# c0gent/hbbft

Hardware: AMD Instinct MI355X
Metric: verified BLS sig shares/sec (whole node) + combine latency, N=64 f=21 (higher is better)
Workload: dtype u32 limbs (Fp, 14x28-bit); 1 GPU; ThresholdSign share verification, BASELINE configs[1]; batch_per_gpu=65536, streams=2, documents_per_gpu=1024, n_nodes=64, f=21, pairing_impl=auto, parallelism=shard-by-batch x1

## Files before the change

### hbbft_amd/csrc/pfp.hpp

```cpp
#pragma once
#include "sfp.hpp"
#include "words.hpp"

#ifndef HP_INV_MODE
#define HP_INV_MODE 0
#endif

#define HP_D __device__ __forceinline__

namespace hbs {

constexpr int DPP_SWAP = 0xB1;
constexpr int DPP_EVEN = 0xA0;
constexpr int DPP_ODD = 0xF5;

HP_D bool lp_even() { return (threadIdx.x & 1) == 0; }
template <int CTRL>
HP_D int32_t dpp(int32_t v) {
  return __builtin_amdgcn_mov_dpp(v, CTRL, 0xF, 0xF, true);
}
template <int CTRL>
HP_D Fp dpp_fp(const Fp& a) {
  Fp r;
#pragma unroll
  for (int i = 0; i < NL; i++) r.l[i] = dpp<CTRL>(a.l[i]);
  return r;
}

HS_MULFN Fp h_mul_l(HS_P14(x), HS_P14(y)) {
  const Fp a = {{HS_L14(x)}};
  const Fp b = {{HS_L14(y)}};
  const int32_t sm = lp_even() ? -1 : 0;
  int32_t Y[NL], W[NL], Z[NL];
#pragma unroll
  for (int i = 0; i < NL; i++) {
    Y[i] = dpp<DPP_EVEN>(b.l[i]);
    W[i] = dpp<DPP_ODD>(b.l[i]);
    Z[i] = (dpp<DPP_SWAP>(a.l[i]) ^ sm) - sm;
  }
  int32_t m[NL];
  int64_t acc = 0;
  Fp r;
#pragma unroll
  for (int k = 0; k < NL; k++) {
#pragma unroll
    for (int i = 0; i <= k; i++) {
      acc += (int64_t)a.l[i] * Y[k - i];
      acc += (int64_t)Z[i] * W[k - i];
    }
#pragma unroll
    for (int i = 0; i < k; i++) acc += (int64_t)m[i] * (int32_t)P_L[k - i];
    m[k] = mont_digit(acc);
    acc += (int64_t)m[k] * (int32_t)P_L[0];
    acc >>= 28;
  }
#pragma unroll
  for (int k = NL; k < 2 * NL - 1; k++) {
#pragma unroll
    for (int i = k - NL + 1; i < NL; i++) {
      acc += (int64_t)a.l[i] * Y[k - i];
      acc += (int64_t)Z[i] * W[k - i];
      acc += (int64_t)m[i] * (int32_t)P_L[k - i];
    }
    r.l[k - NL] = (int32_t)acc & MASK28;
    acc >>= 28;
  }
  r.l[NL - 1] = (int32_t)acc;
  return r;
}

HP_D Fp h_mul(const Fp& a, const Fp& b) { return h_mul_l(HS_E14(a), HS_E14(b)); }

HP_D Fp h_sqr(const Fp& a) {
  const bool ev = lp_even();
  const Fp pa = dpp_fp<DPP_SWAP>(a);
  Fp x, y;
#pragma unroll
  for (int i = 0; i < NL; i++) {
    x.l[i] = pa.l[i] + (ev ? a.l[i] : pa.l[i]);
    y.l[i] = a.l[i] - (ev ? pa.l[i] : 0);
  }
  return fp_mul(x, y);
}

HP_D Fp h_mul_xi(const Fp& a) {
  const int32_t sm = lp_even() ? -1 : 0;
  const Fp pa = dpp_fp<DPP_SWAP>(a);
  Fp r;
#pragma unroll
  for (int i = 0; i < NL; i++) r.l[i] = a.l[i] + ((pa.l[i] ^ sm) - sm);
  fp_norm(r);
  return r;
}
HP_D Fp h_conj(const Fp& a) {
  const Fp n = fp_neg(a);
  return lp_even() ? a : n;
}
HP_D Fp h_zero() { return fp_zero(); }
HP_D Fp h_one() { return lp_even() ? fp_one() : fp_zero(); }
HP_D Fp h_const(const uint32_t (&c0)[NL], const uint32_t (&c1)[NL]) {
  Fp r;
  const bool ev = lp_even();
#pragma unroll
  for (int i = 0; i < NL; i++) r.l[i] = (int32_t)(ev ? c0[i] : c1[i]);
  return r;
}
HP_D bool lp_both(bool v) { return (v ? 1 : 0) & dpp<DPP_SWAP>(v ? 1 : 0); }
HP_D bool h_is_zero(const Fp& a) { return lp_both(fp_is_zero(a)); }
constexpr int INV_PAIR = 8;
template <int N>
HP_D void lp_inv_uniform(const uint32_t* y, const uint32_t* mod, uint32_t* out) {
  static_assert(N <= 15, "words_reduce_32m");
  const bool ev = lp_even();
  uint32_t mine[N], other[N], co[N + 1];
#pragma unroll
  for (int i = 0; i < N; i++) {
    mine[i] = ev ? y[i] : mod[i];
    other[i] = ev ? mod[i] : y[i];
    co[i] = 0;
  }
  co[N] = 0;
  co[0] = ev ? 1u : 0u;
  uint32_t inv = mod[0];
  for (int k = 0; k < 5; k++) inv *= 2u - mod[0] * inv;
  const uint32_t minv = 0u - inv;
  const int rounds = (2 * hb::words_bitlen<N>(mod) - 1 + 30) / 31;
#pragma unroll 1
  for (int r = 0; r < rounds; r++) {
    const uint64_t am = hb::words_approx<N>(mine, hb::words_len2<N>(mine, other));
    const uint64_t ao = (uint64_t)(uint32_t)dpp<DPP_SWAP>((int32_t)(uint32_t)am) |
                        ((uint64_t)(uint32_t)dpp<DPP_SWAP>((int32_t)(uint32_t)(am >> 32)) << 32);
    uint64_t ab = ev ? am : ao, bb = ev ? ao : am;
    uint32_t c0 = ev ? 1u : 0u, c1 = ev ? 0u : 1u;
#pragma unroll 1
    for (int j = 0; j < 31; j++) {
      uint32_t odd;
      bool sw;
      hb::words_divstep_ab(ab, bb, odd, sw);
      hb::words_divstep_col(c0, c1, odd, sw);
    }
    uint32_t km, ks, sm, ss;
    hb::words_fac_split(ev ? c0 : c1, km, ks);
    hb::words_fac_split(ev ? c1 : c0, sm, ss);
    {
      uint32_t t[N + 2], k[N + 2], row[N + 1];
      hb::words_mul_sm<N, false>(mine, sm, ss, t);
#pragma unroll
      for (int i = 0; i < N + 2; i++) t[i] = (uint32_t)dpp<DPP_SWAP>((int32_t)t[i]);
      hb::words_mul_sm<N, false>(mine, km, ks, k);
      uint64_t c = 0;
#pragma unroll
      for (int i = 0; i < N + 2; i++) {
        c += (uint64_t)k[i] + t[i];
        t[i] = (uint32_t)c;
        c >>= 32;
      }
#pragma unroll
      for (int i = 0; i <= N; i++) row[i] = (t[i] >> 31) | (t[i + 1] << 1);
      const uint32_t fl = hb::words_abs<N + 1>(row);
      ks ^= fl;
      ss ^= (uint32_t)dpp<DPP_SWAP>((int32_t)fl);
#pragma unroll
      for (int i = 0; i < N; i++) {
        mine[i] = row[i];
        other[i] = (uint32_t)dpp<DPP_SWAP>((int32_t)row[i]);
      }
    }
    {
      uint32_t t[N + 2], w[N + 2];
      hb::words_mul_sm<N, true>(co, sm, ss, t);
#pragma unroll
      for (int i = 0; i < N + 2; i++) t[i] = (uint32_t)dpp<DPP_SWAP>((int32_t)t[i]);
      const uint32_t xe = 0u - (co[N] >> 31);
      const uint32_t k0 = km & ks;
      const uint64_t q = (uint64_t)(((k0 + (co[0] ^ ks) * km + t[0]) * minv) & 0x7fffffffu);
      uint64_t c = k0;
#pragma unroll
      for (int i = 0; i < N + 2; i++) {
        const uint32_t xi = (i <= N ? co[i] : xe) ^ ks;
        c += (uint64_t)xi * km;
        if (i < N) c += q * mod[i];
        c += t[i];
        w[i] = (uint32_t)c;
        c >>= 32;
      }
#pragma unroll
      for (int i = 0; i <= N; i++) co[i] = (w[i] >> 31) | (w[i + 1] << 1);
    }
  }
  const uint32_t mine_one = hb::words_is_one<N>(mine) ? 1u : 0u;
  const uint32_t part_one = (uint32_t)dpp<DPP_SWAP>((int32_t)mine_one);
  const bool one = (ev ? part_one : mine_one) != 0;
  uint32_t v[N + 1];
#pragma unroll
  for (int i = 0; i <= N; i++) {
    const uint32_t pv = (uint32_t)dpp<DPP_SWAP>((int32_t)co[i]);
    v[i] = ev ? pv : co[i];
  }
  hb::words_reduce_32m<N>(v, mod);
#pragma unroll
  for (int i = 0; i < N; i++) out[i] = one ? v[i] : 0u;
}

template <int MODE = 0>
HP_D Fp h_inv_vartime(const Fp& a) {
  const Fp s = fp_sqr(a);
  const Fp n = fp_add(s, dpp_fp<DPP_SWAP>(s));
  uint32_t w[12], p[12], r[12];
  fp_to_words(n, w);
  uint32_t nz = 0;
#pragma unroll
  for (int i = 0; i < 12; i++) nz |= w[i];
  if (nz == 0) return fp_zero();
#pragma unroll
  for (int i = 0; i < 12; i++) p[i] = hb::PM2_W[i];
  p[0] += 2;
  if ((MODE & INV_PAIR) != 0)
    lp_inv_uniform<12>(w, p, r);
  else
    hb::words_inv_vartime<12, MODE>(w, p, r);
  return h_conj(fp_mul(a, fp_from_words(r)));
}

template <int M, int K>
HP_D Fp fp_red_mk(const Fp& t, const Fp& a) {
  const int64_t top = (int64_t)t.l[NL - 1] * M + (int64_t)K * a.l[NL - 1];
  const int32_t q = (int32_t)((top * QINV) >> 32);
  Fp r;
  int64_t acc = 0;
#pragma unroll
  for (int i = 0; i < NL - 1; i++) {
    acc += (int64_t)t.l[i] * M + (int64_t)K * a.l[i] - (int64_t)q * (int32_t)P_L[i];
    r.l[i] = (int32_t)acc & MASK28;
    acc >>= 28;
  }
  r.l[NL - 1] = (int32_t)(acc + top - (int64_t)q * (int32_t)P_L[NL - 1]);
  return r;
}
HP_D Fp fp_red_l(const Fp& t) { return fp_red_mk<1, 0>(t, t); }
HP_D Fp fp_red_124(const Fp& a, const Fp& b, const Fp& c) {
  const int32_t top = a.l[NL - 1] + 2 * b.l[NL - 1] + 4 * c.l[NL - 1];
  const int32_t q = (int32_t)(((int64_t)top * QINV) >> 32);
  Fp r;
  int64_t acc = 0;
#pragma unroll
  for (int i = 0; i < NL - 1; i++) {
    acc += (int64_t)(a.l[i] + 2 * b.l[i] + 4 * c.l[i]) - (int64_t)q * (int32_t)P_L[i];
    r.l[i] = (int32_t)acc & MASK28;
    acc >>= 28;
  }
  r.l[NL - 1] = (int32_t)(acc + top - (int64_t)q * (int32_t)P_L[NL - 1]);
  return r;
}
HP_D Fp fp_lin3(const Fp& a, int k1, const Fp& b, int k2, const Fp& c) {
  Fp r;
#pragma unroll
  for (int i = 0; i < NL; i++) r.l[i] = a.l[i] + k1 * b.l[i] + k2 * c.l[i];
  fp_norm(r);
  return r;
}
HP_D Fp h_add_xi_l(const Fp& s, const Fp& t) {
  const int32_t sm = lp_even() ? -1 : 0;
  const Fp pt = dpp_fp<DPP_SWAP>(t);
  Fp r;
#pragma unroll
  for (int i = 0; i < NL; i++) r.l[i] = s.l[i] + t.l[i] + ((pt.l[i] ^ sm) - sm);
  return r;
}
HP_D Fp fp_sub2l(const Fp& a, const Fp& b, const Fp& c) {
  Fp r;
#pragma unroll
  for (int i = 0; i < NL; i++) r.l[i] = a.l[i] - b.l[i] - c.l[i];
  return r;
}

HP_D Fp h_xi_l(const Fp& t) {
  const int32_t sm = lp_even() ? -1 : 0;
  const Fp pt = dpp_fp<DPP_SWAP>(t);
  Fp r;
#pragma unroll
  for (int i = 0; i < NL; i++) r.l[i] = t.l[i] + ((pt.l[i] ^ sm) - sm);
  return r;
}

struct H6 { Fp c0, c1, c2; };
struct H12 { H6 c0, c1; };

HP_D H6 h6_zero() { return {h_zero(), h_zero(), h_zero()}; }
HP_D H6 h6_one() { return {h_one(), h_zero(), h_zero()}; }
HP_D H6 h6_add(const H6& a, const H6& b) { return {fp_add(a.c0, b.c0), fp_add(a.c1, b.c1), fp_add(a.c2, b.c2)}; }
HP_D H6 h6_sub(const H6& a, const H6& b) { return {fp_sub(a.c0, b.c0), fp_sub(a.c1, b.c1), fp_sub(a.c2, b.c2)}; }
HP_D H6 h6_neg(const H6& a) { return {fp_neg(a.c0), fp_neg(a.c1), fp_neg(a.c2)}; }
HP_D H6 h6_red(const H6& a) { return {fp_reduce(a.c0), fp_reduce(a.c1), fp_reduce(a.c2)}; }
HP_D H6 h6_mul_v(const H6& a) { return {h_mul_xi(a.c2), a.c0, a.c1}; }

HP_D H6 h6_mul(const H6& a, const H6& b) {
  const Fp v1 = h_mul(a.c1, b.c1);
  const Fp v2 = h_mul(a.c2, b.c2);
  const Fp d0 = fp_sub2l(h_mul(fp_addl(a.c1, a.c2), fp_add(b.c1, b.c2)), v1, v2);
  const Fp v0 = h_mul(a.c0, b.c0);
  const Fp c0 = fp_red_l(h_add_xi_l(v0, d0));
  const Fp c1 = fp_red_l(h_add_xi_l(fp_sub2l(h_mul(fp_addl(a.c0, a.c1), fp_add(b.c0, b.c1)), v0, v1), v2));
  const Fp c2 = fp_red_l(fp_addl(fp_sub2l(h_mul(fp_addl(a.c0, a.c2), fp_add(b.c0, b.c2)), v0, v2), v1));
  return {c0, c1, c2};
}
HP_D H6 h6_mul6(const H6& a, const H6& b) {
  Fp c2, m, e, k, h;
  {
    const Fp sa = fp_add(a.c0, a.c2);
    const Fp p1 = h_mul(fp_addl(sa, a.c1), fp_lin3(b.c0, 1, b.c1, 1, b.c2));
    const Fp pm = h_mul(fp_subl(sa, a.c1), fp_lin3(b.c0, -1, b.c1, 1, b.c2));
    const Fp p0 = h_mul(a.c0, b.c0);
    const Fp pi = h_mul(a.c2, b.c2);
    const Fp xpi = h_xi_l(pi);
    Fp w;
#pragma unroll
    for (int i = 0; i < NL; i++) {
      w.l[i] = p1.l[i] + pm.l[i] - 2 * p0.l[i] - 2 * pi.l[i];
      m.l[i] = 3 * (p0.l[i] - p1.l[i]) - pm.l[i];
      e.l[i] = p1.l[i] - pm.l[i];
      k.l[i] = p0.l[i] - 2 * xpi.l[i];
      h.l[i] = 2 * pi.l[i] + xpi.l[i];
    }
    c2 = fp_red_mk<3, 0>(w, w);
  }
  const Fp t = fp_addl(h_mul(fp_red_124(a.c0, a.c1, a.c2), fp_lin3(b.c0, 2, b.c1, 4, b.c2)), m);
  const Fp c0 = fp_red_mk<1, 6>(h_xi_l(t), k);
  Fp g;
#pragma unroll
  for (int i = 0; i < NL; i++) g.l[i] = 3 * e.l[i] - t.l[i];
  const Fp c1 = fp_red_mk<1, 6>(g, h);
  return {c0, c1, c2};
}
HP_D H6 h6_inv(const H6& a) {
  const Fp c0 = fp_reduce(fp_sub(h_sqr(a.c0), h_mul_xi(h_mul(a.c1, a.c2))));
  const Fp c1 = fp_reduce(fp_sub(h_mul_xi(h_sqr(a.c2)), h_mul(a.c0, a.c1)));
  const Fp c2 = fp_reduce(fp_sub(h_sqr(a.c1), h_mul(a.c0, a.c2)));
  const Fp t = fp_reduce(fp_add(h_mul(a.c0, c0), h_mul_xi(fp_add(h_mul(a.c2, c1), h_mul(a.c1, c2)))));
  const Fp ti = fp_reduce(h_inv_vartime<HP_INV_MODE>(t));
  return {h_mul(c0, ti), h_mul(c1, ti), h_mul(c2, ti)};
}

HP_D H12 h12_one() { return {h6_one(), h6_zero()}; }
HP_D H12 h12_conj(const H12& a) { return {a.c0, h6_neg(a.c1)}; }
HP_D H12 h12_red(const H12& a) { return {h6_red(a.c0), h6_red(a.c1)}; }
HP_D H12 h12_kcomb(const H6& t0, const H6& t1, const H6& s) {
  return {{fp_red_l(h_add_xi_l(t0.c0, t1.c2)), fp_red_l(fp_addl(t0.c1, t1.c0)), fp_red_l(fp_addl(t0.c2, t1.c1))},
          {fp_red_l(fp_sub2l(s.c0, t0.c0, t1.c0)), fp_red_l(fp_sub2l(s.c1, t0.c1, t1.c1)),
           fp_red_l(fp_sub2l(s.c2, t0.c2, t1.c2))}};
}

template <int S = 1>
HP_D H6 h6_mul_12(const H6& x, const Fp& b1, const Fp& b2) {
  const Fp u = h_mul(x.c1, b1);
  const Fp w = h_mul(x.c2, b2);
  const Fp d0 = h_xi_l(fp_sub2l(h_mul(fp_addl(x.c1, x.c2), fp_add(b1, b2)), u, w));
  const Fp c0 = fp_red_mk<S, 0>(d0, d0);
  const Fp d1 = h_add_xi_l(h_mul(x.c0, b1), w);
  const Fp c1 = fp_red_mk<S, 0>(d1, d1);
  const Fp d2 = fp_addl(h_mul(x.c0, b2), u);
  const Fp c2 = fp_red_mk<S, 0>(d2, d2);
  return {c0, c1, c2};
}

HP_D const H6& h6_of(const H6& a) { return a; }
template <class F>
HP_D auto h6_of(const F& f) -> decltype(f()) { return f(); }

template <class G>
HP_D H12 h12_mul(const H12& a, const H12& b) {
  H6 t0, t1;
  G::mul6x2(a.c0, b.c0, a.c1, b.c1, t0, t1);
  const H6 s = G::mul6(h6_add(a.c0, a.c1), h6_add(b.c0, b.c1));
  return h12_kcomb(t0, t1, s);
}
template <class G>
HP_D H12 h12_sqr(const H12& a) {
  H6 t, s;
  const auto a1 = [&]() HS_LAMBDA { return h6_add(a.c0, a.c1); };
  const auto b1 = [&]() HS_LAMBDA { return h6_red(h6_add(a.c0, h6_mul_v(a.c1))); };
  G::miller_mul6x2(a.c0, a.c1, a1, b1, t, s);
  return {{fp_red_l(h_add_xi_l(fp_subl(s.c0, t.c0), fp_subl(fp_zero(), t.c2))), fp_red_l(fp_sub2l(s.c1, t.c1, t.c0)),
           fp_red_l(fp_sub2l(s.c2, t.c2, t.c1))},
          {fp_red_l(fp_addl(t.c0, t.c0)), fp_red_l(fp_addl(t.c1, t.c1)), fp_red_l(fp_addl(t.c2, t.c2))}};
}
template <class G>
HP_D H12 h12_mul_lines(const H12& f, const Fp& a0, const Fp& a1, const Fp& a4, const Fp& b0, const Fp& b1,
                       const Fp& b4, bool first = false) {
  H6 C0, t0, t1;
  Fp c11, c12;
  G::line_product(a0, a1, a4, b0, b1, b4, C0, c11, c12);
  if (first) return {C0, {h_zero(), c11, c12}};
  G::miller_mul6x2_12(f.c0, C0, f.c1, c11, c12, t0, t1);
  const H6 s = G::miller_mul6(h6_add(f.c0, f.c1), {C0.c0, fp_add(C0.c1, c11), fp_add(C0.c2, c12)});
  return h12_kcomb(t0, t1, s);
}
template <class G>
HP_D H12 h12_inv(const H12& a) {
  H6 s0, s1, r0, r1;
  G::mul6x2(a.c0, a.c0, a.c1, a.c1, s0, s1);
  const H6 t = h6_red(h6_sub(h6_red(s0), h6_red(h6_mul_v(h6_red(s1)))));
  const H6 ti = h6_red(h6_inv(t));
  G::mul6x2(a.c0, ti, a.c1, ti, r0, r1);
  return h12_red({r0, h6_neg(r1)});
}

#define HP_FROB1(K) h_const(hb::FROB1_##K##_C0, hb::FROB1_##K##_C1)
HP_D H12 h12_frob1(const H12& f) {
  H12 r;
  r.c0.c0 = h_conj(f.c0.c0);
  r.c1.c0 = h_mul(h_conj(f.c1.c0), HP_FROB1(1));
  r.c0.c1 = h_mul(h_conj(f.c0.c1), HP_FROB1(2));
  r.c1.c1 = h_mul(h_conj(f.c1.c1), HP_FROB1(3));
  r.c0.c2 = h_mul(h_conj(f.c0.c2), HP_FROB1(4));
  r.c1.c2 = h_mul(h_conj(f.c1.c2), HP_FROB1(5));
  return h12_red(r);
}
HP_D H12 h12_frob2(const H12& f) {
  H12 r;
  r.c0.c0 = f.c0.c0;
  r.c1.c0 = fp_mul(f.c1.c0, fp_const(hb::FROB2_1_C0));
  r.c0.c1 = fp_mul(f.c0.c1, fp_const(hb::FROB2_2_C0));
  r.c1.c1 = fp_mul(f.c1.c1, fp_const(hb::FROB2_3_C0));
  r.c0.c2 = fp_mul(f.c0.c2, fp_const(hb::FROB2_4_C0));
  r.c1.c2 = fp_mul(f.c1.c2, fp_const(hb::FROB2_5_C0));
  return r;
}

HP_D H12 h12_cyclo_sqr(const H12& f) {
  const Fp& a0 = f.c0.c0; const Fp& a2 = f.c0.c1; const Fp& a4 = f.c0.c2;
  const Fp& a1 = f.c1.c0; const Fp& a3 = f.c1.c1; const Fp& a5 = f.c1.c2;
  H12 r;
  {
    const Fp s0 = h_sqr(a0), s3 = h_sqr(a3), s03 = h_sqr(fp_add(a0, a3));
    r.c0.c0 = fp_red_mk<3, -2>(h_add_xi_l(s0, s3), a0);
    r.c1.c1 = fp_red_mk<3, 2>(fp_sub2l(s03, s0, s3), a3);
  }
  {
    const Fp s1 = h_sqr(a1), s4 = h_sqr(a4), s14 = h_sqr(fp_add(a1, a4));
    r.c0.c1 = fp_red_mk<3, -2>(h_add_xi_l(s1, s4), a2);
    r.c1.c2 = fp_red_mk<3, 2>(fp_sub2l(s14, s1, s4), a5);
  }
  {
    const Fp s2 = h_sqr(a2), s5 = h_sqr(a5), s25 = h_sqr(fp_add(a2, a5));
    r.c0.c2 = fp_red_mk<3, -2>(h_add_xi_l(s2, s5), a4);
    r.c1.c0 = fp_red_mk<3, 2>(h_add_xi_l(fp_zero(), fp_sub2l(s25, s2, s5)), a1);
  }
  return r;
}

struct HC { Fp a1, a2, a4, a5; };

HP_D HC hc_compress(const H12& f) { return {f.c1.c0, f.c0.c1, f.c0.c2, f.c1.c2}; }
HP_D HC hc_sqr(const HC& c) {
  HC r;
  {
    const Fp s1 = h_sqr(c.a1), s4 = h_sqr(c.a4), s14 = h_sqr(fp_add(c.a1, c.a4));
    r.a2 = fp_red_mk<3, -2>(h_add_xi_l(s1, s4), c.a2);
    r.a5 = fp_red_mk<3, 2>(fp_sub2l(s14, s1, s4), c.a5);
  }
  {
    const Fp s2 = h_sqr(c.a2), s5 = h_sqr(c.a5), s25 = h_sqr(fp_add(c.a2, c.a5));
    r.a4 = fp_red_mk<3, -2>(h_add_xi_l(s2, s5), c.a4);
    r.a1 = fp_red_mk<3, 2>(h_add_xi_l(fp_zero(), fp_sub2l(s25, s2, s5)), c.a1);
  }
  return r;
}
HP_D Fp hc_denom(const Fp& a1) { return fp_lin(4, a1, 0, a1); }
HP_D H12 hc_decompress(const HC& c, const Fp& di) {
  const Fp s5 = h_sqr(c.a5), s2 = h_sqr(c.a2);
  Fp t = h_xi_l(s5);
#pragma unroll
  for (int i = 0; i < NL; i++) t.l[i] += 3 * s2.l[i];
  const Fp a3 = h_mul(fp_red_mk<1, -2>(t, c.a4), di);
  const Fp u = fp_addl(fp_lin(2, h_sqr(a3), -3, h_mul(c.a4, c.a2)), h_mul(c.a1, c.a5));
  const Fp a0 = fp_red_l(h_add_xi_l(h_one(), u));
  return {{a0, c.a2, c.a4}, {c.a1, a3, c.a5}};
}

HP_D bool h12_is_one(const H12& f) {
  bool ok = fp_is_zero(fp_sub(f.c0.c0, h_one()));
  ok = ok && fp_is_zero(f.c0.c1) && fp_is_zero(f.c0.c2);
  ok = ok && fp_is_zero(f.c1.c0) && fp_is_zero(f.c1.c1) && fp_is_zero(f.c1.c2);
  return lp_both(ok);
}

struct HJac { Fp x, y, z; };
struct HLine { Fp c0, c1, c4; };

struct HProj { Fp x, y, z; };

HP_D HLine h_dbl_step_h(HProj& T) {
  const Fp C = h_sqr(T.z);
  const Fp YZ = h_sqr(fp_add(T.y, T.z));
  const Fp B = h_sqr(T.y);
  const Fp H = fp_sub(fp_sub(YZ, B), C);
  const Fp E = fp_red_mk<12, 0>(h_xi_l(C), C);
  const Fp A = h_mul(T.x, T.y);
  const Fp S = h_sqr(T.x);
  HLine l;
  l.c0 = fp_red_mk<1, -1>(B, E);
  l.c1 = fp_lin(-3, S, 0, S);
  l.c4 = H;
  const Fp Bm = fp_lin(1, B, -3, E);
  const Fp Bp = fp_lin(1, B, 3, E);
  T.x = h_mul(fp_addl(A, A), Bm);
  const Fp EE = h_sqr(E);
  T.y = fp_red_mk<1, -12>(h_sqr(Bp), EE);
  const Fp BH = h_mul(fp_addl(B, B), H);
  T.z = fp_red_mk<2, 0>(BH, BH);
  return l;
}

HP_D HLine h_add_step_h(HProj& T, const Fp& xQ, const Fp& yQ) {
  const Fp th = fp_sub(T.y, h_mul(yQ, T.z));
  const Fp la = fp_sub(T.x, h_mul(xQ, T.z));
  HLine l;
  l.c0 = fp_reduce(fp_sub(h_mul(th, xQ), h_mul(la, yQ)));
  l.c1 = fp_neg(th);
  l.c4 = la;
  const Fp C = h_sqr(th);
  const Fp D = h_sqr(la);
  const Fp E = h_mul(la, D);
  const Fp F = h_mul(T.z, C);
  const Fp G = h_mul(T.x, D);
  const Fp H = fp_lin(1, fp_addl(E, F), -2, G);
  const Fp X3 = h_mul(la, H);
  T.y = fp_reduce(fp_sub(h_mul(th, fp_sub(G, H)), h_mul(E, T.y)));
  T.z = h_mul(T.z, E);
  T.x = X3;
  return l;
}

template <class PT>
struct SideStateT {
  Fp xP, yP;
  bool act;
  bool qinf;
  uint32_t q;
  PT T;
};

template <bool GEN, class ST>
HP_D Fp side_xP(const ST& st) { return GEN ? fp_const(hb::G1X_M) : st.xP; }
template <bool GEN, class ST>
HP_D Fp side_yP(const ST& st, bool negate) {
  return GEN ? (negate ? fp_neg(fp_const(hb::G1Y_M)) : fp_const(hb::G1Y_M)) : st.yP;
}

struct NoPark {
  HP_D explicit NoPark(uint32_t*) {}
  template <class ST>
  HP_D void init(const ST&, const ST&) const {}
  template <int SIDE, class ST, class F>
  HP_D HLine walk(ST& st, const F& f) const { return f(st.T); }
  template <int SIDE, class ST>
  HP_D Fp xP(const ST& st) const { return st.xP; }
  template <int SIDE, class ST>
  HP_D Fp yP(const ST& st) const { return st.yP; }
};

constexpr int PARK_WORDS = 72;
constexpr int park_fit(int used, bool need, int words) { return need && used + words <= PARK_WORDS ? used : -1; }
typedef volatile __attribute__((address_space(3))) uint32_t* ParkCol;

HP_D void park_put(ParkCol c, int slot, const Fp& a) {
#pragma unroll
  for (int i = 0; i < NL; i++) c[(slot + i) * 256] = (uint32_t)a.l[i];
}
HP_D Fp park_get(ParkCol c, int slot) {
  Fp r;
#pragma unroll
  for (int i = 0; i < NL; i++) r.l[i] = (int32_t)c[(slot + i) * 256];
  return r;
}

template <bool W1, bool W2, int GEN>
struct PairPark {
  static constexpr int TW = 3 * NL, PW = 2 * NL;
  static constexpr int T_B = park_fit(0, W2, TW);
  static constexpr int U1 = T_B < 0 ? 0 : TW;
  static constexpr int T_A = park_fit(U1, W1, TW);
  static constexpr int U2 = U1 + (T_A < 0 ? 0 : TW);
  static constexpr int P_A = park_fit(U2, GEN != 1, PW);
  static constexpr int U3 = U2 + (P_A < 0 ? 0 : PW);
  static constexpr int P_B = park_fit(U3, GEN != 2, PW);
  template <int SIDE>
  static constexpr int t_slot() { return SIDE == 0 ? T_A : T_B; }
  template <int SIDE>
  static constexpr int p_slot() { return SIDE == 0 ? P_A : P_B; }

  ParkCol col;
  HP_D explicit PairPark(uint32_t* c) : col((ParkCol)c) {}

  template <int SIDE>
  HP_D void put_T(const HProj& T) const {
    park_put(col, t_slot<SIDE>(), T.x);
    park_put(col, t_slot<SIDE>() + NL, T.y);
    park_put(col, t_slot<SIDE>() + 2 * NL, T.z);
  }
  template <int SIDE, class ST>
  HP_D void init_side(const ST& st) const {
    if constexpr (t_slot<SIDE>() >= 0) put_T<SIDE>(st.T);
    if constexpr (p_slot<SIDE>() >= 0) {
      park_put(col, p_slot<SIDE>(), st.xP);
      park_put(col, p_slot<SIDE>() + NL, st.yP);
    }
  }
  template <class ST>
  HP_D void init(const ST& A, const ST& B) const {
    init_side<0>(A);
    init_side<1>(B);
  }
  template <int SIDE, class ST, class F>
  HP_D HLine walk(ST& st, const F& f) const {
    if constexpr (t_slot<SIDE>() < 0) {
      return f(st.T);
    } else {
      HProj T;
      T.z = park_get(col, t_slot<SIDE>() + 2 * NL);
      T.y = park_get(col, t_slot<SIDE>() + NL);
      T.x = park_get(col, t_slot<SIDE>());
      const HLine l = f(T);
      put_T<SIDE>(T);
      return l;
    }
  }
  template <int SIDE, class ST>
  HP_D Fp xP(const ST& st) const {
    if constexpr (p_slot<SIDE>() < 0) return st.xP; else return park_get(col, p_slot<SIDE>());
  }
  template <int SIDE, class ST>
  HP_D Fp yP(const ST& st) const {
    if constexpr (p_slot<SIDE>() < 0) return st.yP; else return park_get(col, p_slot<SIDE>() + NL);
  }
};

struct LanePair {
  static constexpr int LANES = 2;
  static HP_D bool leader() { return lp_even(); }
  static HP_D bool value_writer() { return true; }
  using Walk = HProj;
  static HP_D HLine dbl_step(HProj& T) { return h_dbl_step_h(T); }
  static HP_D HLine add_step(HProj& T, const Fp& xQ, const Fp& yQ) { return h_add_step_h(T, xQ, yQ); }

  static HP_D H6 mul6(const H6& a, const H6& b) { return h6_mul(a, b); }
  template <class A1, class B1>
  static HP_D void mul6x2(const H6& a0, const H6& b0, const A1& a1, const B1& b1, H6& r0, H6& r1) {
    r0 = h6_mul(a0, b0);
    r1 = h6_mul(h6_of(a1), h6_of(b1));
  }
  static HP_D void mul6x2_12(const H6& a0, const H6& b0, const H6& a1, const Fp& c1, const Fp& c2, H6& r0, H6& r1) {
    r0 = h6_mul(a0, b0);
    r1 = h6_mul_12(a1, c1, c2);
  }
  static constexpr int MILLER_SCALE = 6;
  static HP_D H6 miller_mul6(const H6& a, const H6& b) { return h6_mul6(a, b); }
  template <class A1, class B1>
  static HP_D void miller_mul6x2(const H6& a0, const H6& b0, const A1& a1, const B1& b1, H6& r0, H6& r1) {
    r0 = h6_mul6(a0, b0);
    r1 = h6_mul6(h6_of(a1), h6_of(b1));
  }
  static HP_D void miller_mul6x2_12(const H6& a0, const H6& b0, const H6& a1, const Fp& c1, const Fp& c2, H6& r0,
                                    H6& r1) {
    r0 = h6_mul6(a0, b0);
    r1 = h6_mul_12<MILLER_SCALE>(a1, c1, c2);
  }
  template <bool W1, bool W2>
  static constexpr bool first_line() { return W1 || W2; }
  static HP_D void line_product(const Fp& a0, const Fp& a1, const Fp& a4, const Fp& b0, const Fp& b1, const Fp& b4,
                                H6& C0, Fp& c11, Fp& c12) {
    const Fp a0b0 = h_mul(a0, b0);
    const Fp a1b1 = h_mul(a1, b1);
    const Fp a4b4 = h_mul(a4, b4);
    c11 = fp_red_l(fp_sub2l(h_mul(fp_addl(a0, a4), fp_add(b0, b4)), a0b0, a4b4));
    c12 = fp_red_l(fp_sub2l(h_mul(fp_addl(a1, a4), fp_add(b1, b4)), a1b1, a4b4));
    C0 = {fp_red_l(h_add_xi_l(a0b0, a4b4)), fp_red_l(fp_sub2l(h_mul(fp_addl(a0, a1), fp_add(b0, b1)), a0b0, a1b1)),
          a1b1};
  }
  static HP_D H12 cyclo_sqr(const H12& f) { return h12_cyclo_sqr(f); }
  static HP_D H12 frob1(const H12& f) { return h12_frob1(f); }
  static HP_D H12 frob2(const H12& f) { return h12_frob2(f); }

  template <bool W1, bool W2, int GEN>
  using Park = PairPark<W1, W2, GEN>;

  template <bool GEN, int SIDE, class ST, class PK>
  static HP_D HLine line_at_p(const HLine& l, const ST& st, bool negate, const PK& pk) {
    HLine e;
    e.c0 = st.act ? l.c0 : h_one();
    const Fp c1 = fp_mul(l.c1, GEN ? side_xP<true>(st) : pk.template xP<SIDE>(st));
    e.c1 = st.act ? c1 : fp_zero();
    const Fp c4 = fp_mul(l.c4, GEN ? side_yP<true>(st, negate) : pk.template yP<SIDE>(st));
    e.c4 = st.act ? c4 : fp_zero();
    return e;
  }
  template <bool G1, bool G2, bool WALK_FIRST, class RA, class RB, class ST, class PK>
  static HP_D void lines_at_p(const RA& raw_a, const RB& raw_b, const ST& A, const ST& B, bool neg2, HLine& la,
                              HLine& lb, const PK& pk) {
    if constexpr (WALK_FIRST) {
      lb = line_at_p<G2, 1>(raw_b(), B, neg2, pk);
      la = line_at_p<G1, 0>(raw_a(), A, false, pk);
    } else {
      la = line_at_p<G1, 0>(raw_a(), A, false, pk);
      lb = line_at_p<G2, 1>(raw_b(), B, neg2, pk);
    }
  }
};

HP_D void h_g2_load(const uint32_t* __restrict__ w, Fp& x, Fp& y) {
  const int o = lp_even() ? 0 : 12;
  x = fp_from_words(w + o);
  y = fp_from_words(w + 24 + o);
}
HP_D bool words_zero(const uint32_t* __restrict__ w, int n) {
  uint32_t o = 0;
  for (int k = 0; k < n; k++) o |= w[k];
  return o == 0;
}

}
```

Measured before the change: 3.863 million shares/s.

## Fuse Fp4 squaring triples into one interleaved Montgomery product in cyclotomic squaring

```diff
diff --git a/hbbft_amd/csrc/pfp.hpp b/hbbft_amd/csrc/pfp.hpp
--- a/hbbft_amd/csrc/pfp.hpp
+++ b/hbbft_amd/csrc/pfp.hpp
@@ -82,6 +82,90 @@
   }
   return fp_mul(x, y);
 }
+
+#ifndef HP_SQR4
+#define HP_SQR4 1
+#endif
+#if HP_SQR4
+typedef int32_t V28 __attribute__((ext_vector_type(2 * NL)));
+
+HS_MULFN V28 h_sqr4_l(HS_P14(x), HS_P14(y)) {
+  const Fp a = {{HS_L14(x)}};
+  const Fp b = {{HS_L14(y)}};
+  const int32_t sm = lp_even() ? -1 : 0;
+  int32_t xa[NL], ya[NL], xb[NL], yb[NL], xs[NL], ys[NL];
+#pragma unroll
+  for (int i = 0; i < NL; i++) {
+    const int32_t pa = dpp<DPP_SWAP>(a.l[i]), pb = dpp<DPP_SWAP>(b.l[i]);
+    xa[i] = dpp<DPP_EVEN>(a.l[i]) + pa;
+    ya[i] = a.l[i] - (pa & sm);
+    xb[i] = dpp<DPP_EVEN>(b.l[i]) + pb;
+    yb[i] = b.l[i] - (pb & sm);
+    xs[i] = xa[i] + xb[i];
+    ys[i] = ya[i] + yb[i];
+  }
+  int32_t mA[NL], mC[NL], A[NL], C[NL];
+  int64_t cb = 0, ra = 0, rc = 0;
+#pragma unroll
+  for (int k = 0; k < 2 * NL - 1; k++) {
+#pragma unroll
+    for (int i = (k < NL ? 0 : k - NL + 1); i <= (k < NL ? k : NL - 1); i++) {
+      ra += (int64_t)xa[i] * ya[k - i];
+      cb += (int64_t)xb[i] * yb[k - i];
+      rc += (int64_t)xs[i] * ys[k - i];
+    }
+    const int32_t lb = (int32_t)cb & MASK28;
+    cb >>= 28;
+    const int32_t w = (dpp<DPP_SWAP>(lb) ^ sm) - sm;
+    ra += lb + w;
+    rc += w;
+    if (k < NL) {
+#pragma unroll
+      for (int i = 0; i < k; i++) {
+        ra += (int64_t)mA[i] * (int32_t)P_L[k - i];
+        rc += (int64_t)mC[i] * (int32_t)P_L[k - i];
+      }
+      mA[k] = mont_digit(ra);
+      mC[k] = mont_digit(rc);
+      ra += (int64_t)mA[k] * (int32_t)P_L[0];
+      rc += (int64_t)mC[k] * (int32_t)P_L[0];
+    } else {
+#pragma unroll
+      for (int i = k - NL + 1; i < NL; i++) {
+        ra += (int64_t)mA[i] * (int32_t)P_L[k - i];
+        rc += (int64_t)mC[i] * (int32_t)P_L[k - i];
+      }
+      A[k - NL] = (int32_t)ra & MASK28;
+      C[k - NL] = (int32_t)rc & MASK28;
+    }
+    ra >>= 28;
+    rc >>= 28;
+  }
+  const int32_t tb = (int32_t)cb;
+  const int32_t tw = (dpp<DPP_SWAP>(tb) ^ sm) - sm;
+  A[NL - 1] = (int32_t)ra + tb + tw;
+  C[NL - 1] = (int32_t)rc + tw;
+  V28 r;
+#pragma unroll
+  for (int i = 0; i < NL; i++) {
+    r[i] = A[i];
+    r[NL + i] = C[i] - A[i];
+  }
+  return r;
+}
+
+struct Sq4 { Fp A, B; };
+HP_D Sq4 h_sqr4(const Fp& a, const Fp& b) {
+  const V28 v = h_sqr4_l(HS_E14(a), HS_E14(b));
+  Sq4 r;
+#pragma unroll
+  for (int i = 0; i < NL; i++) {
+    r.A.l[i] = v[i];
+    r.B.l[i] = v[NL + i];
+  }
+  return r;
+}
+#endif
 
 HP_D Fp h_mul_xi(const Fp& a) {
   const int32_t sm = lp_even() ? -1 : 0;
@@ -431,6 +515,23 @@
   const Fp& a0 = f.c0.c0; const Fp& a2 = f.c0.c1; const Fp& a4 = f.c0.c2;
   const Fp& a1 = f.c1.c0; const Fp& a3 = f.c1.c1; const Fp& a5 = f.c1.c2;
   H12 r;
+#if HP_SQR4
+  {
+    const Sq4 s = h_sqr4(a0, a3);
+    r.c0.c0 = fp_red_mk<3, -2>(s.A, a0);
+    r.c1.c1 = fp_red_mk<3, 2>(s.B, a3);
+  }
+  {
+    const Sq4 s = h_sqr4(a1, a4);
+    r.c0.c1 = fp_red_mk<3, -2>(s.A, a2);
+    r.c1.c2 = fp_red_mk<3, 2>(s.B, a5);
+  }
+  {
+    const Sq4 s = h_sqr4(a2, a5);
+    r.c0.c2 = fp_red_mk<3, -2>(s.A, a4);
+    r.c1.c0 = fp_red_mk<3, 2>(h_add_xi_l(fp_zero(), s.B), a1);
+  }
+#else
   {
     const Fp s0 = h_sqr(a0), s3 = h_sqr(a3), s03 = h_sqr(fp_add(a0, a3));
     r.c0.c0 = fp_red_mk<3, -2>(h_add_xi_l(s0, s3), a0);
@@ -446,6 +547,7 @@
     r.c0.c2 = fp_red_mk<3, -2>(h_add_xi_l(s2, s5), a4);
     r.c1.c0 = fp_red_mk<3, 2>(h_add_xi_l(fp_zero(), fp_sub2l(s25, s2, s5)), a1);
   }
+#endif
   return r;
 }
 
@@ -454,6 +556,18 @@
 HP_D HC hc_compress(const H12& f) { return {f.c1.c0, f.c0.c1, f.c0.c2, f.c1.c2}; }
 HP_D HC hc_sqr(const HC& c) {
   HC r;
+#if HP_SQR4
+  {
+    const Sq4 s = h_sqr4(c.a1, c.a4);
+    r.a2 = fp_red_mk<3, -2>(s.A, c.a2);
+    r.a5 = fp_red_mk<3, 2>(s.B, c.a5);
+  }
+  {
+    const Sq4 s = h_sqr4(c.a2, c.a5);
+    r.a4 = fp_red_mk<3, -2>(s.A, c.a4);
+    r.a1 = fp_red_mk<3, 2>(h_add_xi_l(fp_zero(), s.B), c.a1);
+  }
+#else
   {
     const Fp s1 = h_sqr(c.a1), s4 = h_sqr(c.a4), s14 = h_sqr(fp_add(c.a1, c.a4));
     r.a2 = fp_red_mk<3, -2>(h_add_xi_l(s1, s4), c.a2);
@@ -464,6 +578,7 @@
     r.a4 = fp_red_mk<3, -2>(h_add_xi_l(s2, s5), c.a4);
     r.a1 = fp_red_mk<3, 2>(h_add_xi_l(fp_zero(), fp_sub2l(s25, s2, s5)), c.a1);
   }
+#endif
   return r;
 }
 HP_D Fp hc_denom(const Fp& a1) { return fp_lin(4, a1, 0, a1); }
```

Result: faster. 3.951 million shares/s (median of 6 runs) (+2.3%).
